# facebookresearch/sound-spaces

Hardware: AMD Instinct MI355X
Metric: audio env-steps/sec (RIR-convolve+spectrogram) per node, 128 envs Replica 16 kHz (higher is better)
Workload: dtype f32

## Files before the change

### include/ss_hip.h

```cpp
#ifndef SS_HIP_H
#define SS_HIP_H

#include <stddef.h>

#ifdef __cplusplus
extern "C" {
#endif

#define SS_EINVAL (-1)
#define SS_PAD_REFLECT 0
#define SS_PAD_CONSTANT 1
#define SS_FLAG_NO_DISTRACTOR 1
#define SS_FLAG_CROSSFADE 2
#define SS_FLAG_FIRST_BUCKET 4

int ss_block_len(void);
int ss_spec_floats(void);
int ss_version(void);

int ss_init(void);
int ss_release_scratch(void);

int ss_source_windows_f32(const float* src, const int* win_desc, float* spec_out, int n_windows,
                          void* stream);
// ... 202 lines not shown
    int* free_slots;
    int n_free;
    float* bank;
    long long bank_unit_stride;
    int bank_chan_stride, cap;
    int* dev_len;
    int* host_len;
    unsigned char* clipped;
    unsigned char* spec_stale;
    int keep;
    float* stage;
    int* stage_slot;
    int* stage_len;
    int* stage_desc;
    int stage_rows, threads;
    const unsigned char* used;
    const long long* use_seq;
    int* evicted_slot;
    int n_evicted, evict_cap;
    long long* loaded_key;
    int* loaded_slot;
    int* loaded_frames;
    int n_loaded, loaded_cap;
} ss_miss_loader;
int ss_ctx_observe_requests_load(ss_ctx* ctx, const long long* recs, int n, ss_request_tables* tables, ss_miss_loader* loader,
                                 float* audiogoal, float* spectrogram, int* miss_out, int* n_miss, void* stream);
int ss_ctx_load_rir_files(ss_ctx* ctx, ss_miss_loader* loader, const char* const* paths, int k, long long* last_used,
                          long long tick, int n_slots, void* stream);
int ss_ctx_requests_units(ss_ctx* ctx, const long long* recs, int n, const ss_request_tables* tables, int* units_out,
                          int* miss_out, int* n_miss);
int ss_ctx_plan(ss_ctx* ctx, const ss_units* units, int n, int* unit_desc_out, int* flags_out, int* n_new_windows_out,
                int* new_windows_out, int new_windows_cap);
int ss_ctx_stats(ss_ctx* ctx, long long* out8);

int ss_wav_read_rirs_f32(const char* const* paths, int n, float* dst, long long row_stride, int cap, int keep, int planar,
                         int* kept_out, int* frames_out, int* status_out, int n_threads);
int ss_bank_scatter_rows_f32(const float* staged, long long staged_row_stride, const int* slots, const int* lens, int n,
                             float* bank, long long unit_stride, int chan_stride, int cap, int* bank_len, void* stream);
int ss_bank_scatter_spectra_f32(const float* staged, long long staged_row_stride, int planar, const int* slots, const int* lens,
                                int n, float* hspec, int h_blocks, int* bank_len, void* stream);
int ss_bank_scatter_spectra16_f32(const float* staged, long long staged_row_stride, int planar, const int* slots, const int* lens,
                                  int n, void* hspec16, float* hscale, int h_blocks, int* bank_len, void* stream);
int ss_rows_gather_f32(const float* const* src, const int* n_floats, int n, float* dst, long long row_stride, int row_floats,
                       int n_threads);

#ifdef __cplusplus
}
#endif
#endif
```

### sound-spaces_amd/build.py

```python
#!/usr/bin/env python
import os
import subprocess
import sys

HERE = os.path.dirname(os.path.abspath(__file__))
CSRC = os.path.join(HERE, "csrc")
SO = os.path.join(CSRC, "libss_hip.so")
TORCH_SO = os.path.join(CSRC, "libss_torch_ops.so")
SOURCES = ["ss_torch_ops.cpp", "ss_hip.hip", "ss_kernels.hpp", "ss_fft_core.hpp", "ss_kernels32.hpp", "ss_fft_core32.hpp", "ss_features.hpp", "ss_tables.hpp", "ss_context.hpp", "ss_wavio.hpp", os.path.join("..", "..", "include", "ss_hip.h")]
FLAGS = ["--offload-arch=gfx950", "-O3", "-std=c++17", "-fPIC", "-shared", "-Wall", "-Wno-unused-function"]


STAMP = os.path.join(CSRC, ".libss_hip.srchash")
KERNEL_SOURCES = [s for s in SOURCES if s != "ss_torch_ops.cpp"]
KERNEL_STAMP = os.path.join(CSRC, ".libss_hip.kernelhash")


def _source_hash(sources=None):
    import hashlib
    h = hashlib.sha256(" ".join(FLAGS).encode())
    for s in (SOURCES if sources is None else sources):
        with open(os.path.join(CSRC, s), "rb") as f:
            h.update(f.read())
    return h.hexdigest()


def kernel_hash():
    return _source_hash(KERNEL_SOURCES)


def up_to_date():
    if not (os.path.exists(SO) and os.path.exists(STAMP)):
        return False
    if not os.path.exists(TORCH_SO) and not os.path.exists(TORCH_SO + ".skipped"):
        return False
    return open(STAMP).read().strip() == _source_hash()


def build(force=False, verbose=True):
    build_bench_token(force, verbose)
    if not force and up_to_date():
        if not os.path.exists(KERNEL_STAMP):
# ... 83 lines not shown
```

### sound-spaces_amd/csrc/ss_context.hpp

```cpp
#pragma once
#include <hip/hip_runtime.h>

#include <cstdint>
#include <cstring>
#include <unordered_map>
#include <vector>

#include "../../include/ss_hip.h"

namespace ssctx {

constexpr int kDirectDescUnits = 256;
constexpr int kRing = 16;
constexpr int kGroup = 4;
constexpr int kGuardTicks = 8;
constexpr int kLanes = 4;

inline int ceil_div(int a, int b) { return (a + b - 1) / b; }
inline int hip_rc(hipError_t e) { return e == hipSuccess ? 0 : -static_cast<int>(e); }

struct WindowSet {
    int m_min = 0, count = 0;
};

inline WindowSet plan_window_set(int source_len, long long t0, int nbh_max, int nby, bool wrap, int kb) {
    const long long limit = wrap ? 2LL * source_len : source_len;
    WindowSet ws;
    bool any = false;
    for (int m = -(nbh_max - 1); m <= nby - 1; ++m) {
        if (t0 + (long long)(m + 1) * kb > 0 && t0 + (long long)(m - 1) * kb < limit) {
            if (!any) { ws.m_min = m; any = true; }
            ++ws.count;
        }
    }
    return ws;
}

struct Entry {
    uint64_t key = 0;
    int m_min = 0, count = 0;
    long long tick = -1;
// ... 3 lines not shown

struct Context {
    int sr = 0, n_valid = 0, out_len = 0, pad_mode = 0, wrap_mode = 0, kb = 0, spec_floats = 0;
    int device = 0;
    float* src_dev = nullptr;
    size_t src_cap = 0, src_used = 0;
    std::vector<int> src_off, src_len;
    const float* rir = nullptr;
    const int* rir_len = nullptr;
    long long rir_us = 0;
    int rir_cs = 0, rir_es = 1, rir_cap = 0;
    const float* hspec = nullptr;
    const float* hscale = nullptr;
    int h_blocks = 0;
    std::vector<ss_rir_bucket> buckets;
    std::vector<ss_spec_bucket> spec_buckets;
    int stride = 1;
    int n_entries = 0;
    int pool_entries = 0;
    float* pool = nullptr;
    std::vector<Entry> entries;
    std::unordered_map<uint64_t, int> map;
    int lru_head = -1, lru_tail = -1;
    std::vector<int> free_list;
    long long tick = 0;
    long long hits = 0, misses = 0, evictions = 0, grows = 0;
    int ring_cap = 0, ring_k = 0;
    int* h_desc = nullptr;
    int* d_desc = nullptr;
    int win_cap = 0;
    int* h_win = nullptr;
    int* d_win = nullptr;
    hipEvent_t ev_done[kRing / kGroup] = {};
    bool group_open = false;
    int open_group = 0;
    hipStream_t group_stream = nullptr;
    bool ev_made = false;
    float* ag_scratch = nullptr;
    size_t ag_cap = 0;
    std::vector<int> sim_scratch;
    std::vector<int> new_win;
    std::vector<int> new_entries;
    bool plan_only_keys = false;
    hipStream_t last_stream = nullptr;
    bool have_last_stream = false;
    hipEvent_t ev_xstream = nullptr;
    int n_lanes = 1, lane_next = 0;
    void* miss_ev = nullptr;
    int spectral_max_units = 0;
    int mel_fused_min_units = 1, mel_fused_max_units = 0x7fffffff;
    int mel_rows_min_units = 1, mel_rows_max_units = 0;
    int mel_ss2_min_units = 1, mel_ss2_max_units = 0;
    int chip_share = 0;
    hipStream_t lane_stream[kLanes] = {};
    bool lane_dirty[kLanes] = {};
    bool lane_joined[kLanes] = {};
    bool lane_join_valid[kLanes] = {};
    hipStream_t lane_join_stream[kLanes] = {};
    hipEvent_t ev_lane[kLanes] = {};
    hipEvent_t ev_in = nullptr;
    hipEvent_t ev_win[kLanes] = {};
    long long win_seq[kLanes] = {};
    long long win_seen[kLanes][kLanes] = {};
    hipEvent_t ev_done_l[kLanes][kRing / kGroup] = {};
    bool lanes_made = false;
};

inline uint64_t make_key(int sound, long long t0, bool wrap) {
    return (static_cast<uint64_t>(static_cast<uint32_t>(sound)) << 33) |
// ... 172 lines not shown
```

### sound-spaces_amd/csrc/ss_hip.hip

```cpp
#include <hip/hip_runtime.h>

#include <algorithm>
#include <chrono>
#include <cstdlib>
#include <iterator>
#include <map>
#include <mutex>
#include <utility>
#include <new>
#include <string>
#include <vector>

#include "../../include/ss_hip.h"
#include "ss_context.hpp"
#include "ss_kernels.hpp"
#include "ss_kernels32.hpp"
#include "ss_features.hpp"
#include "ss_tables.hpp"
#include "ss_wavio.hpp"

namespace {

constexpr int kMaxDevices = 64;
struct DeviceTables {
// ... 39 lines not shown
    hipError_t e = hipGetDevice(&dev);
    if (e != hipSuccess) return hip_err(e);
    if (dev < 0 || dev >= kMaxDevices) return SS_EINVAL;
    std::lock_guard<std::mutex> lk(g_mu);
    DeviceTables& d = g_tables[dev];
    if (!d.ready) {
        const std::vector<float> host = ssk_host::build_tables();
        float* dev_buf = nullptr;
        e = hipMalloc(&dev_buf, host.size() * sizeof(float));
        if (e != hipSuccess) return hip_err(e);
        e = hipMemcpy(dev_buf, host.data(), host.size() * sizeof(float), hipMemcpyHostToDevice);
        if (e != hipSuccess) { (void)hipFree(dev_buf); return hip_err(e); }
        d.tb.twM = reinterpret_cast<const ssk::c32*>(dev_buf + ssk_host::kTwMOff);
        d.tb.twItem = reinterpret_cast<const ssk::c32*>(dev_buf + ssk_host::kTwItemOff);
        d.tb.tw512 = reinterpret_cast<const ssk::c32*>(dev_buf + ssk_host::kTw512Off);
        d.tb.win = dev_buf + ssk_host::kWinOff;
        d.tb.twG = reinterpret_cast<const ssk::c32*>(dev_buf + ssk_host::kTwGOff);
        d.tb.twP2 = reinterpret_cast<const ssk::c32*>(dev_buf + ssk_host::kTwP2Off);
        int cus = 0;
        e = hipDeviceGetAttribute(&cus, hipDeviceAttributeMultiprocessorCount, dev);
        if (e != hipSuccess) { (void)hipFree(dev_buf); return hip_err(e); }
        d.n_cus = cus > 0 ? cus : 1;
        d.ready = true;
    }
    *out = d.tb;
    if (n_cus) *n_cus = d.n_cus;
    return 0;
}

inline int n_frames_of(int len) { return 1 + len / ssk::kHop; }
inline int t4_of(int len) { return (n_frames_of(len) + ssk::kPool - 1) / ssk::kPool; }

thread_local const int* g_host_desc = nullptr;
thread_local int g_launch_share = 1;

inline bool fill_unit_tab(ssk::UnitTab<true>& ut, const int* host_desc, int n_units) {
    if (!host_desc || n_units > ssk::kTabUnits) return false;
    static const bool no_sort = ab_flag("SS_HIP_NO_SORT");
    unsigned key[ssk::kTabUnits];
    bool sortable = !no_sort && n_units >= 64;
    for (int i = 0; i < n_units; ++i) {
        const int* d = host_desc + 8 * i;
        const bool ok = d[0] >= 0 && d[2] <= 0 && d[2] + d[3] > 0;
        const int slot = ok ? d[1] - d[2] : 0xffffff;
        if (slot < 0 || slot > 0xffffff) sortable = false;
        key[i] = (static_cast<unsigned>(slot & 0xffffff) << 8) | static_cast<unsigned>(i);
    }
    if (sortable) std::sort(key, key + n_units);
    for (int k = 0; k < n_units; ++k) {
        const int i = sortable ? static_cast<int>(key[k] & 0xffu) : k;
        const int* d = host_desc + 8 * i;
        const bool ok = d[0] >= 0 && d[2] <= 0 && d[2] + d[3] > 0;
        ut.tab[ssk::kTabWords * k] = ok ? d[0] : -1;
        ut.tab[ssk::kTabWords * k + 1] = ok ? d[1] - d[2] : 0;
        ut.tab[ssk::kTabWords * k + 2] = i;
    }
    return true;
}

inline bool wide_one_block_ok(int out_len, int n_valid, int flags, bool spectral = false) {
    static const bool off = ab_flag("SS_HIP_NO_WIDE");
    if (off || spectral || out_len <= ssk::kB || n_valid < 0 || n_valid > ssk::kB) return false;
    if ((flags & SS_FLAG_CROSSFADE) &&
        (static_cast<int>(0.05 * out_len) < 1 || static_cast<int>(0.05 * out_len) > 2 * ssk::kPrevPairs - 2)) return false;
    return ssk::live_blocks(n_valid, out_len, t4_of(out_len)) <= 26;
}

inline int parts_log2_for(int n_rows, int n_cus) {
    static const int forced = ab_int("SS_HIP_PARTS_LOG2", -1);
    if (forced >= 0) return forced < 3 ? forced : 3;
    const int cus = n_cus / (g_launch_share > 1 ? g_launch_share : 1);
    int k = 0;
    while (k < 3 && (n_rows << (k + 1)) <= cus) ++k;
    return k;
}

template <bool FUSE>
int launch_conv(ssk::ConvParams p, int n_units, int nb_y, int flags, int n_cus, hipStream_t st, bool wide = false) {
    if (nb_y < 1 || nb_y > 3 || (FUSE && nb_y != 1)) return SS_EINVAL;
    p.nb_y = nb_y;
    p.parts_log2 = FUSE && !wide ? parts_log2_for(2 * n_units, n_cus) : 0;
    if constexpr (FUSE) {
        if (wide) {
            if ((flags & SS_FLAG_CROSSFADE) && (p.fade_len < 1 || p.fade_len > 2 * ssk::kPrevPairs - 2)) return SS_EINVAL;
            const dim3 grid(2 * n_units, 1), block(ssk::kT);
            if (flags & SS_FLAG_CROSSFADE)
                hipLaunchKernelGGL((ssk::k_conv<true, false, true, false, true>), grid, block, 0, st, p, ssk::UnitTab<false>());
            else
                hipLaunchKernelGGL((ssk::k_conv<true, false, false, false, true>), grid, block, 0, st, p, ssk::UnitTab<false>());
// ... 1044 lines not shown
    return launch_obs_rows<true, true, true>(p, n_units, flags, n_cus, static_cast<hipStream_t>(stream), m, ssk::SpecScale<true>{hscale});
}

struct ss_ctx { ssctx::Context c; };

int ss_ctx_create(ss_ctx** out, int sampling_rate, int n_valid, int pad_mode, int wrap_mode, int max_window_sets) {
    if (!out || sampling_rate <= 0 || n_valid < 0 || n_valid > sampling_rate || n_valid > 3 * ssk::kB) return SS_EINVAL;
    if (pad_mode != SS_PAD_REFLECT && pad_mode != SS_PAD_CONSTANT) return SS_EINVAL;
    ss_ctx* h = new (std::nothrow) ss_ctx();
    if (!h) return SS_EINVAL;
    ssctx::Context& c = h->c;
    c.sr = sampling_rate; c.n_valid = n_valid; c.out_len = sampling_rate; c.pad_mode = pad_mode;
    c.wrap_mode = wrap_mode ? 1 : 0;
    c.kb = ssk::kB; c.spec_floats = 2 * ssk::kSpecComplex;
    c.n_entries = max_window_sets > 0 ? max_window_sets : 256;
    c.stride = n_valid > 0 ? ssctx::ceil_div(n_valid, ssk::kB) : 1;
    ssctx::cache_reset(c);
    *out = h;
    return 0;
}

static void ctx_free_device(ssctx::Context& c) {
    if (c.pool) (void)hipFree(c.pool);
    if (c.src_dev) (void)hipFree(c.src_dev);
    if (c.d_desc) (void)hipFree(c.d_desc);
    if (c.d_win) (void)hipFree(c.d_win);
    if (c.h_desc) (void)hipHostFree(c.h_desc);
    if (c.h_win) (void)hipHostFree(c.h_win);
    if (c.ag_scratch) (void)hipFree(c.ag_scratch);
    c.ag_scratch = nullptr; c.ag_cap = 0;
    drop_wave_scratch(&c);
    if (c.ev_made)
        for (int k = 0; k < ssctx::kRing / ssctx::kGroup; ++k) (void)hipEventDestroy(c.ev_done[k]);
    if (c.ev_xstream) (void)hipEventDestroy(c.ev_xstream);
    if (c.miss_ev) { (void)hipEventDestroy(static_cast<hipEvent_t>(c.miss_ev)); c.miss_ev = nullptr; }
    c.ev_xstream = nullptr; c.have_last_stream = false;
    if (c.lanes_made) {
        for (int l = 0; l < ssctx::kLanes; ++l) {
            (void)hipStreamSynchronize(c.lane_stream[l]);
            drop_stash(c.lane_stream[l]);
            (void)hipEventDestroy(c.ev_lane[l]);
            (void)hipEventDestroy(c.ev_win[l]);
            (void)hipStreamDestroy(c.lane_stream[l]);
        }
        (void)hipEventDestroy(c.ev_in);
        for (int l = 1; l < ssctx::kLanes; ++l)
            for (int k = 0; k < ssctx::kRing / ssctx::kGroup; ++k) (void)hipEventDestroy(c.ev_done_l[l][k]);
        c.lanes_made = false;
    }
    c.pool = nullptr; c.src_dev = nullptr; c.d_desc = nullptr; c.d_win = nullptr; c.h_desc = nullptr; c.h_win = nullptr;
    c.ev_made = false;
}

int ss_ctx_destroy(ss_ctx* h) {
    if (!h) return 0;
    ctx_free_device(h->c);
    delete h;
    return 0;
}

int ss_ctx_add_source(ss_ctx* h, const float* clip, int len, int on_device) {
    if (!h || !clip || len <= 0) return SS_EINVAL;
    ssctx::Context& c = h->c;
    const size_t need = c.src_used + static_cast<size_t>(len);
    if (need > c.src_cap) {
        size_t cap = c.src_cap ? c.src_cap : (1u << 20);
// ... 86 lines not shown
int ss_ctx_set_rir_spectra16_rows(ss_ctx* h, const void* hspec16, const float* hscale, int h_blocks) {
    if (!h) return SS_EINVAL;
    ssctx::Context& c = h->c;
    if (!hspec16) {
        if (c.hscale) { c.hspec = nullptr; c.hscale = nullptr; c.h_blocks = 0; }
        return 0;
    }
    if (!hscale || h_blocks < 1 || h_blocks > 16 || (reinterpret_cast<size_t>(hspec16) & 7)) return SS_EINVAL;
    if (c.out_len <= c.kb || c.out_len > 3 * c.kb) return SS_EINVAL;
    if (c.rir || !c.buckets.empty() || !c.spec_buckets.empty() || !c.rir_len || (c.hspec && !c.hscale)) return SS_EINVAL;
    if (h_blocks != (c.rir_cap > 0 ? ssctx::ceil_div(c.rir_cap, c.kb) : 1)) return SS_EINVAL;
    c.hspec = static_cast<const float*>(hspec16);
    c.hscale = hscale;
    c.h_blocks = h_blocks;
    return 0;
}

int ss_ctx_plan(ss_ctx* h, const ss_units* units, int n, int* unit_desc_out, int* flags_out, int* n_new_windows_out,
                int* new_windows_out, int new_windows_cap) {
    if (!h || !unit_desc_out) return SS_EINVAL;
    ssctx::PlanResult res;
    int rc = ssctx::plan_units(h->c, units, n, unit_desc_out, &res);
    if (rc) return rc;
    h->c.plan_only_keys = true;
    if (flags_out) *flags_out = res.flags;
    if (n_new_windows_out) *n_new_windows_out = res.n_new_windows;
    if (new_windows_out) {
        const int k = res.n_new_windows < new_windows_cap ? res.n_new_windows : new_windows_cap;
        std::memcpy(new_windows_out, h->c.new_win.data(), sizeof(int) * 5 * static_cast<size_t>(k));
    }
    return 0;
}

int ss_ctx_stats(ss_ctx* h, long long* out8) {
    if (!h || !out8) return SS_EINVAL;
    const ssctx::Context& c = h->c;
    out8[0] = c.hits; out8[1] = c.misses; out8[2] = c.evictions; out8[3] = c.grows;
    out8[4] = c.n_entries; out8[5] = static_cast<long long>(c.map.size()); out8[6] = c.stride; out8[7] = c.tick;
    return 0;
}

static int ctx_ensure_ring(ssctx::Context& c, int n, int n_win, hipStream_t st) {
    hipError_t e;
    if (!c.ev_made) {
        for (int k = 0; k < ssctx::kRing / ssctx::kGroup; ++k) {
            e = hipEventCreateWithFlags(&c.ev_done[k], hipEventDisableTiming);
            if (e != hipSuccess) return hip_err(e);
        }
        c.ev_made = true;
    }
    if (n > c.ring_cap) {
        e = hipDeviceSynchronize();
        if (e != hipSuccess) return hip_err(e);
        int cap = c.ring_cap ? c.ring_cap : 256;
        while (cap < n) cap *= 2;
        if (c.h_desc) (void)hipHostFree(c.h_desc);
        if (c.d_desc) (void)hipFree(c.d_desc);
        c.h_desc = nullptr; c.d_desc = nullptr; c.ring_cap = 0;
        const size_t bytes = sizeof(int) * 8 * static_cast<size_t>(cap) * ssctx::kRing;
        e = hipHostMalloc(reinterpret_cast<void**>(&c.h_desc), bytes, hipHostMallocDefault);
        if (e != hipSuccess) return hip_err(e);
        e = hipMalloc(reinterpret_cast<void**>(&c.d_desc), bytes);
        if (e != hipSuccess) return hip_err(e);
        c.ring_cap = cap;
    }
    if (n_win > c.win_cap) {
        e = hipDeviceSynchronize();
        if (e != hipSuccess) return hip_err(e);
        int cap = c.win_cap ? c.win_cap : 256;
        while (cap < n_win) cap *= 2;
        if (c.h_win) (void)hipHostFree(c.h_win);
        if (c.d_win) (void)hipFree(c.d_win);
        c.h_win = nullptr; c.d_win = nullptr; c.win_cap = 0;
        const size_t bytes = sizeof(int) * 5 * static_cast<size_t>(cap) * ssctx::kRing;
        e = hipHostMalloc(reinterpret_cast<void**>(&c.h_win), bytes, hipHostMallocDefault);
        if (e != hipSuccess) return hip_err(e);
        e = hipMalloc(reinterpret_cast<void**>(&c.d_win), bytes);
        if (e != hipSuccess) return hip_err(e);
        c.win_cap = cap;
    }
    (void)st;
// ... 18 lines not shown
}

static int ctx_observe_on(ss_ctx* h, const ss_units* units, int n, float* audiogoal, float* spectrogram, void* stream,
                          int lane, const ss_features* mel = nullptr) {
    ssctx::Context& c = h->c;
    hipStream_t st = static_cast<hipStream_t>(stream);
    hipError_t e;
    SS_PROF_BEGIN();
    if (c.plan_only_keys) {
        e = hipDeviceSynchronize();
        if (e != hipSuccess) return hip_err(e);
        ssctx::cache_reset(c);
        c.plan_only_keys = false;
    }
    if (lane >= 0) {
        for (int o = 0; o < c.n_lanes; ++o) {
            if (o == lane || c.win_seen[lane][o] >= c.win_seq[o]) continue;
            e = hipStreamWaitEvent(st, c.ev_win[o], 0);
            if (e != hipSuccess) return hip_err(e);
            c.win_seen[lane][o] = c.win_seq[o];
        }
    } else if (c.have_last_stream && st != c.last_stream) {
        if (!c.ev_xstream) {
            e = hipEventCreateWithFlags(&c.ev_xstream, hipEventDisableTiming);
            if (e != hipSuccess) return hip_err(e);
        }
        e = hipEventRecord(c.ev_xstream, c.last_stream);
        if (e == hipSuccess) e = hipStreamWaitEvent(st, c.ev_xstream, 0);
        if (e != hipSuccess) return hip_err(e);
    }
    SS_PROF_MARK(1);
    int rc = ctx_ensure_ring(c, n, 0, st);
    if (rc) return rc;
    if (lane < 0 && c.group_open && (st != c.group_stream || c.ring_k / ssctx::kGroup != c.open_group)) {
        e = hipEventRecord(c.ev_done[c.open_group], c.group_stream);
        if (e != hipSuccess) return hip_err(e);
        c.group_open = false;
        c.ring_k = (c.open_group + 1) * ssctx::kGroup % ssctx::kRing;
    }
    const int k = c.ring_k, g = k / ssctx::kGroup;
    if (k % ssctx::kGroup == 0) {
        e = hipEventSynchronize(c.ev_done[g]);
        for (int l = 1; lane >= 0 && l < c.n_lanes && e == hipSuccess; ++l) e = hipEventSynchronize(c.ev_done_l[l][g]);
        if (e != hipSuccess) return hip_err(e);
        c.group_open = lane < 0;
        c.group_stream = st;
        c.open_group = g;
    }
    static const bool force_copy = ab_flag("SS_HIP_DESC_COPY");
    const bool direct = !force_copy && n <= ssctx::kDirectDescUnits;
    int* hd = c.h_desc + static_cast<size_t>(k) * c.ring_cap * 8;
    int* dd = direct ? hd : c.d_desc + static_cast<size_t>(k) * c.ring_cap * 8;
    ssctx::PlanResult res;
    SS_PROF_MARK(2);
    rc = ssctx::plan_units(c, units, n, hd, &res);
    if (rc) return rc;
    const bool spec_bk = !c.spec_buckets.empty();
    if (!c.rir && c.buckets.empty() && ((!c.hspec && !spec_bk) || (res.flags & SS_FLAG_CROSSFADE))) {
        ssctx::cache_rollback(c);
        return SS_EINVAL;
    }
    SS_PROF_MARK(3);
    c.ring_k = (k + 1) % ssctx::kRing;
    auto close_slot = [&]() -> int {
        hipError_t ee = hipSuccess;
        if (lane >= 0) {
            if (k % ssctx::kGroup >= ssctx::kGroup - c.n_lanes) ee = hipEventRecord(lane == 0 ? c.ev_done[g] : c.ev_done_l[lane][g], st);
        } else if (k % ssctx::kGroup == ssctx::kGroup - 1) {
            ee = hipEventRecord(c.ev_done[g], st);
            c.group_open = false;
        }
        return hip_err(ee);
    };
    auto fail = [&](int code) { ssctx::cache_rollback(c); (void)close_slot(); return code; };
    rc = ctx_ensure_pool(c, st);
    if (rc) return fail(rc);
    if (res.n_new_windows > 0) {
        rc = ctx_ensure_ring(c, n, res.n_new_windows, st);
        if (rc) return fail(rc);
        int* hw = c.h_win + static_cast<size_t>(k) * c.win_cap * 5;
        int* dw = c.d_win + static_cast<size_t>(k) * c.win_cap * 5;
        std::memcpy(hw, c.new_win.data(), sizeof(int) * 5 * static_cast<size_t>(res.n_new_windows));
        e = hipMemcpyAsync(dw, hw, sizeof(int) * 5 * static_cast<size_t>(res.n_new_windows), hipMemcpyHostToDevice, st);
        if (e != hipSuccess) return fail(hip_err(e));
        rc = launch_windows_scatter(c.src_dev, dw, c.pool, res.n_new_windows, st);
        if (rc) return fail(rc);
        if (lane >= 0) {
            e = hipEventRecord(c.ev_win[lane], st);
            if (e != hipSuccess) return fail(hip_err(e));
            ++c.win_seq[lane];
        }
    }
    c.new_entries.clear();
    c.last_stream = st;
    c.have_last_stream = true;
    if (!direct) {
        e = hipMemcpyAsync(dd, hd, sizeof(int) * 8 * static_cast<size_t>(n), hipMemcpyHostToDevice, st);
        if (e != hipSuccess) return fail(hip_err(e));
    }
    const bool spectral = (c.hspec || spec_bk) && !(res.flags & SS_FLAG_CROSSFADE) &&
                          !(c.spectral_max_units > 0 && c.rir && c.out_len <= ssk::kB && n > c.spectral_max_units &&
                            (res.flags & SS_FLAG_NO_DISTRACTOR));
    const int nbh_bank = spectral && !spec_bk ? c.h_blocks : (c.rir_cap > 0 ? ssctx::ceil_div(c.rir_cap, c.kb) : 1);
    const bool mel_fused = mel && c.buckets.empty() && !spec_bk && obs_logmel_shape_ok(c.out_len, res.flags) &&
                           n >= c.mel_fused_min_units && n <= c.mel_fused_max_units;
    const bool mel_rows = mel && !mel_fused && (!c.hscale || c.out_len > c.kb) && c.buckets.empty() && !spec_bk && (spectral || (c.rir && c.rir_cap > 0)) &&
                          obs_logmel_rows_shape_ok(c.out_len, c.n_valid, nbh_bank, res.flags) &&
                          n >= c.mel_rows_min_units && n <= c.mel_rows_max_units;
    const bool mel_ss2 = mel && !mel_fused && !mel_rows && c.buckets.empty() && c.rir && !spectral &&
                         obs_logmel_ss2_shape(c.out_len, c.n_valid, res.flags) != 0 &&
                         n >= c.mel_ss2_min_units && n <= c.mel_ss2_max_units;
    if (mel && !mel_fused && !mel_rows && !mel_ss2) {
        rc = get_wave_scratch(&c, lane < 0 ? 0 : lane, st, static_cast<size_t>(n) * 2 * c.out_len, &audiogoal);
        if (rc) return fail(rc);
    }
    if (spectrogram && !audiogoal && !mel_rows && c.out_len > ssk::kB && !wide_one_block_ok(c.out_len, c.n_valid, res.flags, spectral) &&
        !obs_rows_ok(c.out_len, c.n_valid, nbh_bank, res.flags, spectral, true)) {
        const size_t need = static_cast<size_t>(n) * 2 * c.out_len;
        if (need > c.ag_cap) {
            e = hipDeviceSynchronize();
            if (e != hipSuccess) return fail(hip_err(e));
            if (c.ag_scratch) (void)hipFree(c.ag_scratch);
            c.ag_scratch = nullptr; c.ag_cap = 0;
            e = hipMalloc(reinterpret_cast<void**>(&c.ag_scratch), need * sizeof(float));
            if (e != hipSuccess) return fail(hip_err(e));
            c.ag_cap = need;
        }
        audiogoal = c.ag_scratch;
    }
    static const bool no_tab = ab_flag("SS_HIP_NO_UNIT_TAB");
    SS_PROF_MARK(4);
    g_host_desc = no_tab ? nullptr : hd;
    g_launch_share = c.chip_share > 0 ? c.chip_share : c.n_lanes;
    if (mel_ss2) {
        rc = ss_audio_obs_logmel_ss2_f32(c.pool, c.rir, c.rir_len, dd, nullptr, spectrogram, mel->logmel, mel->mel_start, mel->mel_w,
                                         mel->n_mels, mel->max_len, mel->mel_eps, n, c.rir_us, c.rir_cs, c.rir_es, c.rir_cap,
                                         c.n_valid, c.out_len, c.pad_mode, res.flags, stream);
    } else if (mel_rows) {
        rc = spectral && c.hscale
                 ? ss_audio_obs_logmel_rows_spec16_f32(c.pool, c.hspec, c.hscale, c.rir_len, dd, nullptr, spectrogram, mel->logmel,
                                                       mel->mel_start, mel->mel_w, mel->n_mels, mel->max_len, mel->mel_eps, n,
                                                       c.h_blocks, c.n_valid, c.out_len, c.pad_mode, res.flags, stream)
             : spectral ? ss_audio_obs_logmel_rows_spec_f32(c.pool, c.hspec, c.rir_len, dd, nullptr, spectrogram, mel->logmel,
                                                          mel->mel_start, mel->mel_w, mel->n_mels, mel->max_len, mel->mel_eps, n,
                                                          c.h_blocks, c.n_valid, c.out_len, c.pad_mode, res.flags, stream)
                      : ss_audio_obs_logmel_rows_f32(c.pool, c.rir, c.rir_len, dd, nullptr, spectrogram, mel->logmel, mel->mel_start,
                                                     mel->mel_w, mel->n_mels, mel->max_len, mel->mel_eps, n, c.rir_us, c.rir_cs,
                                                     c.rir_es, c.rir_cap, c.n_valid, c.out_len, c.pad_mode, res.flags, stream);
    } else if (mel_fused) {
        rc = spectral && c.hscale
                 ? ss_audio_obs_logmel_spec16_f32(c.pool, c.hspec, c.hscale, c.rir_len, dd, nullptr, spectrogram, mel->logmel,
                                                  mel->mel_start, mel->mel_w, mel->n_mels, mel->max_len, mel->mel_eps, n, c.h_blocks,
                                                  c.n_valid, c.out_len, c.pad_mode, res.flags, stream)
             : spectral ? ss_audio_obs_logmel_spec_f32(c.pool, c.hspec, c.rir_len, dd, nullptr, spectrogram, mel->logmel, mel->mel_start,
                                                     mel->mel_w, mel->n_mels, mel->max_len, mel->mel_eps, n, c.h_blocks, c.n_valid,
                                                     c.out_len, c.pad_mode, res.flags, stream)
                      : ss_audio_obs_logmel_f32(c.pool, c.rir, c.rir_len, dd, nullptr, spectrogram, mel->logmel, mel->mel_start,
                                                mel->mel_w, mel->n_mels, mel->max_len, mel->mel_eps, n, c.rir_us, c.rir_cs, c.rir_es,
                                                c.rir_cap, c.n_valid, c.out_len, c.pad_mode, res.flags, stream);
    } else if (spec_bk) {
        const int nb = static_cast<int>(c.spec_buckets.size());
        rc = spectrogram ? ss_audio_obs_spec_buckets_f32(c.pool, c.spec_buckets.data(), nb, c.rir_len, dd, audiogoal, spectrogram, n,
                                                         c.n_valid, c.out_len, c.pad_mode, res.flags, stream)
                         : ss_fftconv_binaural_spec_buckets_f32(c.pool, c.spec_buckets.data(), nb, c.rir_len, dd, audiogoal, n,
                                                                c.n_valid, c.out_len, res.flags, stream);
    } else if (!c.buckets.empty()) {
        const int nb = static_cast<int>(c.buckets.size());
        rc = spectrogram ? ss_audio_obs_buckets_f32(c.pool, c.buckets.data(), nb, c.rir_len, dd, audiogoal, spectrogram, n,
                                                    c.n_valid, c.out_len, c.pad_mode, res.flags, stream)
                         : ss_fftconv_binaural_buckets_f32(c.pool, c.buckets.data(), nb, c.rir_len, dd, audiogoal, n, c.n_valid,
                                                           c.out_len, res.flags, stream);
    } else if (spectrogram && spectral && c.hscale && c.out_len > c.kb)
        rc = ss_audio_obs_rows_spec16_f32(c.pool, c.hspec, c.hscale, c.rir_len, dd, audiogoal, spectrogram, n, c.h_blocks, c.n_valid,
                                          c.out_len, c.pad_mode, res.flags, stream);
    else if (spectrogram && spectral && c.hscale)
        rc = ss_audio_obs_spec16_f32(c.pool, c.hspec, c.hscale, c.rir_len, dd, audiogoal, spectrogram, n, c.h_blocks, c.n_valid,
                                     c.out_len, c.pad_mode, res.flags, stream);
    else if (spectral && c.hscale)
        rc = ss_fftconv_binaural_spec16_f32(c.pool, c.hspec, c.hscale, c.rir_len, dd, audiogoal, n, c.h_blocks, c.n_valid, c.out_len,
                                            res.flags, stream);
    else if (spectrogram && spectral)
        rc = ss_audio_obs_spec_f32(c.pool, c.hspec, c.rir_len, dd, audiogoal, spectrogram, n, c.h_blocks, c.n_valid,
                                   c.out_len, c.pad_mode, res.flags, stream);
    else if (spectrogram)
        rc = ss_audio_obs_f32(c.pool, c.rir, c.rir_len, dd, audiogoal, spectrogram, n, c.rir_us, c.rir_cs, c.rir_es,
                              c.rir_cap, c.n_valid, c.out_len, c.pad_mode, res.flags, stream);
    else if (spectral)
        rc = ss_fftconv_binaural_spec_f32(c.pool, c.hspec, c.rir_len, dd, audiogoal, n, c.h_blocks, c.n_valid, c.out_len,
                                          res.flags, stream);
    else
        rc = ss_fftconv_binaural_f32(c.pool, c.rir, c.rir_len, dd, audiogoal, n, c.rir_us, c.rir_cs, c.rir_es, c.rir_cap,
                                     c.n_valid, c.out_len, res.flags, stream);
    g_host_desc = nullptr;
    g_launch_share = 1;
    SS_PROF_MARK(5);
    if (!rc && mel && !mel_fused && !mel_rows && !mel_ss2)
        rc = ss_audio_features_f32(audiogoal, n, c.out_len, c.pad_mode, nullptr, mel->logmel, mel->mel_start, mel->mel_w,
                                   mel->n_mels, mel->max_len, mel->mel_eps, nullptr, 1, 1.f, stream);
    if (rc) return fail(rc);
    rc = close_slot();
    SS_PROF_MARK(6);
    return rc;
}

int ss_ctx_set_overlap(ss_ctx* h, int n_streams) {
    if (!h || n_streams < 1 || n_streams > ssctx::kLanes) return SS_EINVAL;
    ssctx::Context& c = h->c;
    hipError_t e = hipDeviceSynchronize();
    if (e != hipSuccess) return hip_err(e);
    if (n_streams > 1 && !c.lanes_made) {
        for (int l = 0; l < ssctx::kLanes; ++l) {
            e = hipStreamCreateWithFlags(&c.lane_stream[l], hipStreamNonBlocking);
            if (e == hipSuccess) e = hipEventCreateWithFlags(&c.ev_lane[l], hipEventDisableTiming);
            if (e == hipSuccess) e = hipEventCreateWithFlags(&c.ev_win[l], hipEventDisableTiming);
            if (e != hipSuccess) return hip_err(e);
        }
        e = hipEventCreateWithFlags(&c.ev_in, hipEventDisableTiming);
        if (e != hipSuccess) return hip_err(e);
        for (int k = 0; k < ssctx::kRing / ssctx::kGroup; ++k) {
            for (int l = 1; l < ssctx::kLanes; ++l) {
                e = hipEventCreateWithFlags(&c.ev_done_l[l][k], hipEventDisableTiming);
                if (e != hipSuccess) return hip_err(e);
            }
        }
        c.lanes_made = true;
    }
    c.n_lanes = n_streams;
    c.lane_next = 0;
    c.ring_k = 0;
    c.group_open = false;
    c.have_last_stream = false;
    for (int l = 0; l < ssctx::kLanes; ++l) { c.lane_dirty[l] = false; c.lane_joined[l] = false; c.lane_join_valid[l] = false; for (int o = 0; o < ssctx::kLanes; ++o) c.win_seen[l][o] = c.win_seq[o]; }
    return 0;
}

int ss_ctx_set_spectral_policy(ss_ctx* h, int max_units) {
    if (!h || max_units < 0) return SS_EINVAL;
    h->c.spectral_max_units = max_units;
    return 0;
}

int ss_ctx_set_logmel_policy(ss_ctx* h, int min_units, int max_units) {
    if (!h || min_units < 0 || max_units < 0) return SS_EINVAL;
    h->c.mel_fused_min_units = min_units;
    h->c.mel_fused_max_units = max_units;
    return 0;
}

int ss_ctx_set_logmel_rows_policy(ss_ctx* h, int min_units, int max_units) {
    if (!h || min_units < 0 || max_units < 0) return SS_EINVAL;
    h->c.mel_rows_min_units = min_units;
    h->c.mel_rows_max_units = max_units;
    return 0;
}

int ss_ctx_set_logmel_ss2_policy(ss_ctx* h, int min_units, int max_units) {
    if (!h || min_units < 0 || max_units < 0) return SS_EINVAL;
    h->c.mel_ss2_min_units = min_units;
    h->c.mel_ss2_max_units = max_units;
    return 0;
}

size_t ss_ctx_wave_scratch_bytes(const ss_ctx* h) {
// ... 871 lines not shown
```

### sound-spaces_amd/ss_amd/_lib.py

```python
from __future__ import annotations

import ctypes
import os

_HERE = os.path.dirname(os.path.abspath(__file__))
SO_PATH = os.path.normpath(os.path.join(_HERE, "..", "csrc", "libss_hip.so"))

EXPORTS = ("ss_block_len", "ss_spec_floats", "ss_version", "ss_init", "ss_source_windows_f32",
           "ss_fftconv_binaural_f32", "ss_spectrogram_f32", "ss_audio_obs_f32", "ss_intensity_f32", "ss_logmel_f32", "ss_gccphat_f32",
           "ss_ctx_create", "ss_ctx_destroy", "ss_ctx_add_source", "ss_ctx_add_source_len", "ss_ctx_set_rir_bank",
           "ss_ctx_observe", "ss_ctx_plan", "ss_ctx_stats", "ss_ctx_set_rir_spectra",
           "ss_rir_spectra_f32", "ss_fftconv_binaural_spec_f32", "ss_audio_obs_spec_f32", "ss_ctx_observe_sims",
           "ss_ctx_sims_units", "ss_ctx_set_overlap", "ss_ctx_join", "ss_fftconv_binaural_buckets_f32",
           "ss_audio_obs_buckets_f32", "ss_ctx_set_rir_buckets", "ss_release_scratch",
           "ss_source_windows32_f32", "ss_audio_obs32_f32", "ss_ctx_observe_requests", "ss_ctx_requests_units", "ss_audio_features_f32", "ss_ctx_observe_features",
           "ss_wav_read_rirs_f32", "ss_rows_gather_f32", "ss_bank_scatter_rows_f32", "ss_ctx_set_chip_share", "ss_ctx_set_spectral_policy", "ss_ctx_observe_requests_load", "ss_ctx_load_rir_files",
           "ss_bank_scatter_spectra_f32", "ss_audio_obs_logmel_f32", "ss_audio_obs_logmel_spec_f32", "ss_ctx_set_logmel_policy",
           "ss_audio_obs_logmel_rows_f32", "ss_audio_obs_logmel_rows_spec_f32", "ss_ctx_set_logmel_rows_policy",
           "ss_audio_obs_logmel_ss2_f32", "ss_ctx_set_logmel_ss2_policy",
           "ss_rir_spectra16_f32", "ss_bank_scatter_spectra16_f32", "ss_fftconv_binaural_spec16_f32", "ss_audio_obs_spec16_f32",
           "ss_audio_obs_logmel_spec16_f32", "ss_ctx_set_rir_spectra16",
           "ss_audio_obs_rows_spec16_f32", "ss_audio_obs_logmel_rows_spec16_f32", "ss_ctx_set_rir_spectra16_rows",
           "ss_fftconv_binaural_spec_buckets_f32", "ss_audio_obs_spec_buckets_f32", "ss_ctx_set_rir_spec_buckets")
EXPORTS_SIZE = ("ss_ctx_wave_scratch_bytes",)


class SsRirBucket(ctypes.Structure):
    _fields_ = [("rir", ctypes.c_void_p), ("hspec", ctypes.c_void_p), ("first", ctypes.c_int), ("n_entries", ctypes.c_int),
                ("cap", ctypes.c_int), ("reserved", ctypes.c_int)]


class SsSpecBucket(ctypes.Structure):
    _fields_ = [("hspec", ctypes.c_void_p), ("hscale", ctypes.c_void_p), ("first", ctypes.c_int), ("n_entries", ctypes.c_int),
                ("cap", ctypes.c_int), ("reserved", ctypes.c_int)]


class SsMissLoader(ctypes.Structure):
    _fields_ = [("table_dirs", ctypes.POINTER(ctypes.c_char_p)), ("n_table_dirs", ctypes.c_int),
                ("pair_keys", ctypes.c_void_p), ("pair_slots", ctypes.c_void_p), ("pair_cap", ctypes.c_int),
                ("free_slots", ctypes.c_void_p), ("n_free", ctypes.c_int),
                ("bank", ctypes.c_void_p), ("bank_unit_stride", ctypes.c_longlong), ("bank_chan_stride", ctypes.c_int),
                ("cap", ctypes.c_int), ("dev_len", ctypes.c_void_p), ("host_len", ctypes.c_void_p), ("clipped", ctypes.c_void_p),
                ("spec_stale", ctypes.c_void_p), ("keep", ctypes.c_int),
                ("stage", ctypes.c_void_p), ("stage_slot", ctypes.c_void_p), ("stage_len", ctypes.c_void_p),
# ... 34 lines not shown
class SsHipError(RuntimeError):
    pass


def load() -> ctypes.CDLL:
    global _lib
    if _lib is not None:
        return _lib
    if not os.path.exists(SO_PATH):
        raise SsHipError(f"{SO_PATH} not found: build it with `python sound-spaces_amd/build.py` "
                         "(or __graft_entry__.build()); there is no CPU fallback for this path")
    lib = ctypes.CDLL(SO_PATH)
    c_int, c_ll, vp = ctypes.c_int, ctypes.c_longlong, ctypes.c_void_p
    lib.ss_block_len.restype = c_int
    lib.ss_spec_floats.restype = c_int
    lib.ss_version.restype = c_int
    lib.ss_init.restype = c_int
    lib.ss_source_windows_f32.argtypes = [vp, vp, vp, c_int, vp]
    lib.ss_fftconv_binaural_f32.argtypes = [vp, vp, vp, vp, vp, c_int, c_ll, c_int, c_int, c_int, c_int, c_int, c_int, vp]
    lib.ss_spectrogram_f32.argtypes = [vp, vp, c_int, c_int, c_int, vp]
    lib.ss_audio_obs_f32.argtypes = [vp, vp, vp, vp, vp, vp, c_int, c_ll, c_int, c_int, c_int, c_int, c_int, c_int, c_int, vp]
    lib.ss_intensity_f32.argtypes = [vp, vp, c_int, c_int, c_int, vp]
    lib.ss_gccphat_f32.argtypes = [vp, vp, c_int, c_int, c_int, c_int, ctypes.c_float, vp]
    lib.ss_logmel_f32.argtypes = [vp, vp, c_int, c_int, c_int, vp, vp, c_int, c_int, ctypes.c_float, vp]
    pp = ctypes.POINTER(ctypes.c_void_p)
    lib.ss_ctx_create.argtypes = [pp, c_int, c_int, c_int, c_int, c_int]
    lib.ss_ctx_destroy.argtypes = [vp]
    lib.ss_ctx_add_source.argtypes = [vp, vp, c_int, c_int]
    lib.ss_ctx_add_source_len.argtypes = [vp, c_int]
    lib.ss_ctx_set_rir_bank.argtypes = [vp, vp, vp, c_ll, c_int, c_int, c_int]
    lib.ss_ctx_observe.argtypes = [vp, ctypes.POINTER(SsUnits), c_int, vp, vp, vp]
    lib.ss_ctx_plan.argtypes = [vp, ctypes.POINTER(SsUnits), c_int, vp, vp, vp, vp, c_int]
    lib.ss_ctx_stats.argtypes = [vp, vp]
    lib.ss_ctx_observe_sims.argtypes = [vp, ctypes.POINTER(SsSimColumns), c_int, vp, vp, vp, vp, vp]
    lib.ss_ctx_sims_units.argtypes = [vp, ctypes.POINTER(SsSimColumns), c_int, vp, vp, vp]
    lib.ss_ctx_set_rir_spectra.argtypes = [vp, vp, c_int]
    lib.ss_ctx_set_overlap.argtypes = [vp, c_int]
    lib.ss_fftconv_binaural_buckets_f32.argtypes = [vp, vp, c_int, vp, vp, vp, c_int, c_int, c_int, c_int, vp]
    lib.ss_audio_obs_buckets_f32.argtypes = [vp, vp, c_int, vp, vp, vp, vp, c_int, c_int, c_int, c_int, c_int, vp]
    lib.ss_ctx_set_rir_buckets.argtypes = [vp, vp, c_int, vp]
    lib.ss_ctx_join.argtypes = [vp, vp]
    lib.ss_ctx_set_chip_share.argtypes = [vp, c_int]
    lib.ss_ctx_set_spectral_policy.argtypes = [vp, c_int]
    lib.ss_rir_spectra_f32.argtypes = [vp, vp, c_int, c_ll, c_int, c_int, vp]
    lib.ss_fftconv_binaural_spec_f32.argtypes = [vp, vp, vp, vp, vp, c_int, c_int, c_int, c_int, c_int, vp]
    lib.ss_audio_obs_spec_f32.argtypes = [vp, vp, vp, vp, vp, vp, c_int, c_int, c_int, c_int, c_int, c_int, vp]
    lib.ss_audio_obs_logmel_f32.argtypes = [vp, vp, vp, vp, vp, vp, vp, vp, vp, c_int, c_int, ctypes.c_float, c_int, c_ll, c_int, c_int,
                                            c_int, c_int, c_int, c_int, c_int, vp]
    lib.ss_audio_obs_logmel_spec_f32.argtypes = [vp, vp, vp, vp, vp, vp, vp, vp, vp, c_int, c_int, ctypes.c_float, c_int, c_int, c_int,
                                                 c_int, c_int, c_int, vp]
    lib.ss_ctx_set_logmel_policy.argtypes = [vp, c_int, c_int]
    lib.ss_audio_obs_logmel_rows_f32.argtypes = lib.ss_audio_obs_logmel_f32.argtypes
    lib.ss_audio_obs_logmel_rows_spec_f32.argtypes = lib.ss_audio_obs_logmel_spec_f32.argtypes
    lib.ss_ctx_set_logmel_rows_policy.argtypes = [vp, c_int, c_int]
    lib.ss_audio_obs_logmel_ss2_f32.argtypes = lib.ss_audio_obs_logmel_f32.argtypes
    lib.ss_ctx_set_logmel_ss2_policy.argtypes = [vp, c_int, c_int]
    lib.ss_ctx_wave_scratch_bytes.argtypes = [vp]
    lib.ss_source_windows32_f32.argtypes = [vp, vp, vp, c_int, vp]
    lib.ss_audio_obs32_f32.argtypes = [vp, vp, vp, vp, vp, vp, c_int, c_ll, c_int, c_int, c_int, c_int, c_int, c_int, vp]
    lib.ss_audio_features_f32.argtypes = [vp, c_int, c_int, c_int, vp, vp, vp, vp, c_int, c_int, ctypes.c_float, vp, c_int,
                                          ctypes.c_float, vp]
    lib.ss_ctx_observe_features.argtypes = [vp, ctypes.POINTER(SsUnits), c_int, vp, vp, ctypes.POINTER(SsFeatures), vp]
    lib.ss_ctx_observe_requests.argtypes = [vp, vp, c_int, vp, vp, vp, vp, vp, vp]
    lib.ss_ctx_requests_units.argtypes = [vp, vp, c_int, vp, vp, vp, vp]
    lib.ss_ctx_observe_requests_load.argtypes = [vp, vp, c_int, vp, vp, vp, vp, vp, vp, vp]
    lib.ss_ctx_load_rir_files.argtypes = [vp, vp, vp, c_int, vp, c_ll, c_int, vp]
# ... 58 lines not shown
```

### sound-spaces_amd/ss_amd/context.py

```python
from __future__ import annotations

import ctypes
from typing import Dict, Optional

import numpy as np

from . import _lib
from .planning import spectrogram_shape

_PAD = {"reflect": 0, "constant": 1, 0: 0, 1: 1}


def _col(a, dtype):
    if a is None:
        return None
    a = np.ascontiguousarray(a, dtype=dtype)
    return a


_NO_MISS = np.zeros((0,), np.int32)


class AudioContext:
    def __init__(self, sampling_rate: int, step_time: Optional[float] = None, wrap: bool = False,
# ... 312 lines not shown
        if rc != 0:
            _lib.check(rc, "ss_ctx_observe_requests")
        return miss["n"].value

    def observe_requests_load(self, recs: bytes, n: int, tables, loader, spectrogram_ptr, audiogoal_ptr, stream: int, miss) -> int:
        rc = self.lib.ss_ctx_observe_requests_load(self._h, recs, n, tables["ref"], loader["ref"], audiogoal_ptr, spectrogram_ptr,
                                                   miss["ptr"], miss["n_ptr"], stream)
        if rc != 0:
            _lib.check(rc, "ss_ctx_observe_requests_load")
        return miss["n"].value

    def requests_units(self, recs: bytes, n: int, tables):
        out = np.zeros((5, max(n, 1)), np.int32)
        miss, n_miss = np.zeros((max(n, 1),), np.int32), ctypes.c_int(0)
        _lib.check(self.lib.ss_ctx_requests_units(self._h, recs, n, tables["ref"], out.ctypes.data, miss.ctypes.data,
                                                  ctypes.addressof(n_miss)), "ss_ctx_requests_units")
        return dict(zip(("sound", "t0", "rir", "dis_sound", "dis_rir"), out[:, :n])), miss[:min(n_miss.value, n)].copy()

    def plan(self, sound, t0, rir, dis_sound=None, dis_rir=None, last_rir=None, wrap=None, last_wrap=None):
        u, n, keep = self._units(sound, t0, rir, dis_sound, dis_rir, last_rir, wrap, last_wrap)
        desc = np.zeros((n, 8), np.int32)
        flags, nw = ctypes.c_int(0), ctypes.c_int(0)
        cap = 2 * self.stats()["slots_per_key"] * n + 16
        wins = np.zeros((cap, 5), np.int32)
        _lib.check(self.lib.ss_ctx_plan(self._h, ctypes.byref(u), n, desc.ctypes.data, ctypes.addressof(flags),
                                        ctypes.addressof(nw), wins.ctypes.data, cap), "ss_ctx_plan")
        assert nw.value <= cap
        return desc, flags.value, wins[:nw.value]

    def stats(self) -> Dict[str, int]:
        out = np.zeros(8, np.int64)
        _lib.check(self.lib.ss_ctx_stats(self._h, out.ctypes.data), "ss_ctx_stats")
        keys = ("hits", "misses", "evictions", "grows", "capacity", "resident", "slots_per_key", "steps")
        return dict(zip(keys, (int(v) for v in out)))
```

Measured before the change: 4.695 million.

## Skip ring-slot release events when slots unread and add pacing event

Moves descriptor-ring group release logic into a Release helper that records a group's done event only if some slot in the group was actually read by the device, and only waits on groups that were recorded. When the unit table was passed by value and no new windows were staged, the slot counts as unread, so the event record and later host synchronize are skipped. A separate Pace event is recorded every kRing steps, with a host wait on the previous one, to bound how far the host runs ahead once ring events stop being recorded. Counters are exposed through a new ring-stats API, and the risk is a subtle reuse hazard if the slot_read tracking misses a case where the device still reads the slot.

```diff
diff --git a/include/ss_hip.h b/include/ss_hip.h
--- a/include/ss_hip.h
+++ b/include/ss_hip.h
@@ -258,6 +258,7 @@
 int ss_ctx_plan(ss_ctx* ctx, const ss_units* units, int n, int* unit_desc_out, int* flags_out, int* n_new_windows_out,
                 int* new_windows_out, int new_windows_cap);
 int ss_ctx_stats(ss_ctx* ctx, long long* out8);
+int ss_ctx_ring_stats(ss_ctx* ctx, long long* out4);
 
 int ss_wav_read_rirs_f32(const char* const* paths, int n, float* dst, long long row_stride, int cap, int keep, int planar,
                          int* kept_out, int* frames_out, int* status_out, int n_threads);
diff --git a/sound-spaces_amd/build.py b/sound-spaces_amd/build.py
--- a/sound-spaces_amd/build.py
+++ b/sound-spaces_amd/build.py
@@ -7,7 +7,7 @@
 CSRC = os.path.join(HERE, "csrc")
 SO = os.path.join(CSRC, "libss_hip.so")
 TORCH_SO = os.path.join(CSRC, "libss_torch_ops.so")
-SOURCES = ["ss_torch_ops.cpp", "ss_hip.hip", "ss_kernels.hpp", "ss_fft_core.hpp", "ss_kernels32.hpp", "ss_fft_core32.hpp", "ss_features.hpp", "ss_tables.hpp", "ss_context.hpp", "ss_wavio.hpp", os.path.join("..", "..", "include", "ss_hip.h")]
+SOURCES = ["ss_torch_ops.cpp", "ss_hip.hip", "ss_kernels.hpp", "ss_fft_core.hpp", "ss_kernels32.hpp", "ss_fft_core32.hpp", "ss_features.hpp", "ss_tables.hpp", "ss_context.hpp", "ss_ring.hpp", "ss_wavio.hpp", os.path.join("..", "..", "include", "ss_hip.h")]
 FLAGS = ["--offload-arch=gfx950", "-O3", "-std=c++17", "-fPIC", "-shared", "-Wall", "-Wno-unused-function"]
 
 
diff --git a/sound-spaces_amd/csrc/ss_context.hpp b/sound-spaces_amd/csrc/ss_context.hpp
--- a/sound-spaces_amd/csrc/ss_context.hpp
+++ b/sound-spaces_amd/csrc/ss_context.hpp
@@ -7,6 +7,7 @@
 #include <vector>
 
 #include "../../include/ss_hip.h"
+#include "ss_ring.hpp"
 
 namespace ssctx {
 
@@ -76,9 +77,10 @@
     int* h_win = nullptr;
     int* d_win = nullptr;
     hipEvent_t ev_done[kRing / kGroup] = {};
-    bool group_open = false;
-    int open_group = 0;
+    ssring::Release<kRing, kGroup> ring;
     hipStream_t group_stream = nullptr;
+    ssring::Pace<kRing> pace;
+    hipEvent_t ev_pace = nullptr;
     bool ev_made = false;
     float* ag_scratch = nullptr;
     size_t ag_cap = 0;
diff --git a/sound-spaces_amd/csrc/ss_hip.hip b/sound-spaces_amd/csrc/ss_hip.hip
--- a/sound-spaces_amd/csrc/ss_hip.hip
+++ b/sound-spaces_amd/csrc/ss_hip.hip
@@ -95,6 +95,7 @@
 inline int t4_of(int len) { return (n_frames_of(len) + ssk::kPool - 1) / ssk::kPool; }
 
 thread_local const int* g_host_desc = nullptr;
+thread_local bool g_tab_taken = false;
 thread_local int g_launch_share = 1;
 
 inline bool fill_unit_tab(ssk::UnitTab<true>& ut, const int* host_desc, int n_units) {
@@ -118,6 +119,7 @@
         ut.tab[ssk::kTabWords * k + 1] = ok ? d[1] - d[2] : 0;
         ut.tab[ssk::kTabWords * k + 2] = i;
     }
+    g_tab_taken = true;
     return true;
 }
 
@@ -1228,6 +1230,7 @@
     drop_wave_scratch(&c);
     if (c.ev_made)
         for (int k = 0; k < ssctx::kRing / ssctx::kGroup; ++k) (void)hipEventDestroy(c.ev_done[k]);
+    if (c.ev_pace) { (void)hipEventDestroy(c.ev_pace); c.ev_pace = nullptr; }
     if (c.ev_xstream) (void)hipEventDestroy(c.ev_xstream);
     if (c.miss_ev) { (void)hipEventDestroy(static_cast<hipEvent_t>(c.miss_ev)); c.miss_ev = nullptr; }
     c.ev_xstream = nullptr; c.have_last_stream = false;
@@ -1380,6 +1383,13 @@
     return 0;
 }
 
+int ss_ctx_ring_stats(ss_ctx* h, long long* out4) {
+    if (!h || !out4) return SS_EINVAL;
+    out4[0] = h->c.ring.n_records; out4[1] = h->c.ring.n_waits;
+    out4[2] = h->c.pace.n_records; out4[3] = h->c.pace.n_waits;
+    return 0;
+}
+
 int ss_ctx_stats(ss_ctx* h, long long* out8) {
     if (!h || !out8) return SS_EINVAL;
     const ssctx::Context& c = h->c;
@@ -1395,6 +1405,8 @@
             e = hipEventCreateWithFlags(&c.ev_done[k], hipEventDisableTiming);
             if (e != hipSuccess) return hip_err(e);
         }
+        e = hipEventCreateWithFlags(&c.ev_pace, hipEventDisableTiming);
+        if (e != hipSuccess) return hip_err(e);
         c.ev_made = true;
     }
     if (n > c.ring_cap) {
@@ -1479,20 +1491,26 @@
     SS_PROF_MARK(1);
     int rc = ctx_ensure_ring(c, n, 0, st);
     if (rc) return rc;
-    if (lane < 0 && c.group_open && (st != c.group_stream || c.ring_k / ssctx::kGroup != c.open_group)) {
-        e = hipEventRecord(c.ev_done[c.open_group], c.group_stream);
+    if (lane < 0 && c.ring.must_close_before(c.ring_k, st == c.group_stream)) {
+        const int og = c.ring.open_group;
+        if (c.ring.close_early()) {
+            e = hipEventRecord(c.ev_done[og], c.group_stream);
+            if (e != hipSuccess) return hip_err(e);
+        }
+        c.ring_k = c.ring.next_slot();
+    }
+    const int k = c.ring_k, g = k / ssctx::kGroup;
+    if (lane < 0) {
+        if (c.ring.begin(k)) {
+            e = hipEventSynchronize(c.ev_done[g]);
+            if (e != hipSuccess) return hip_err(e);
+        }
+        if (k % ssctx::kGroup == 0) c.group_stream = st;
+    } else if (k % ssctx::kGroup == 0) {
+        e = hipEventSynchronize(c.ev_done[g]);
+        for (int l = 1; l < c.n_lanes && e == hipSuccess; ++l) e = hipEventSynchronize(c.ev_done_l[l][g]);
         if (e != hipSuccess) return hip_err(e);
-        c.group_open = false;
-        c.ring_k = (c.open_group + 1) * ssctx::kGroup % ssctx::kRing;
-    }
-    const int k = c.ring_k, g = k / ssctx::kGroup;
-    if (k % ssctx::kGroup == 0) {
-        e = hipEventSynchronize(c.ev_done[g]);
-        for (int l = 1; lane >= 0 && l < c.n_lanes && e == hipSuccess; ++l) e = hipEventSynchronize(c.ev_done_l[l][g]);
-        if (e != hipSuccess) return hip_err(e);
-        c.group_open = lane < 0;
-        c.group_stream = st;
-        c.open_group = g;
+        ++c.ring.n_waits;
     }
     static const bool force_copy = ab_flag("SS_HIP_DESC_COPY");
     const bool direct = !force_copy && n <= ssctx::kDirectDescUnits;
@@ -1509,13 +1527,23 @@
     }
     SS_PROF_MARK(3);
     c.ring_k = (k + 1) % ssctx::kRing;
+    bool slot_read = true;
     auto close_slot = [&]() -> int {
         hipError_t ee = hipSuccess;
         if (lane >= 0) {
-            if (k % ssctx::kGroup >= ssctx::kGroup - c.n_lanes) ee = hipEventRecord(lane == 0 ? c.ev_done[g] : c.ev_done_l[lane][g], st);
-        } else if (k % ssctx::kGroup == ssctx::kGroup - 1) {
+            if (k % ssctx::kGroup >= ssctx::kGroup - c.n_lanes) {
+                ee = hipEventRecord(lane == 0 ? c.ev_done[g] : c.ev_done_l[lane][g], st);
+                ++c.ring.n_records;
+            }
+        } else if (c.ring.end(k, slot_read)) {
             ee = hipEventRecord(c.ev_done[g], st);
-            c.group_open = false;
+            c.pace.ring_event();
+        } else {
+            bool wait_first = false;
+            if (c.pace.step(&wait_first)) {
+                if (wait_first) ee = hipEventSynchronize(c.ev_pace);
+                if (ee == hipSuccess) ee = hipEventRecord(c.ev_pace, st);
+            }
         }
         return hip_err(ee);
     };
@@ -1578,6 +1606,7 @@
     static const bool no_tab = ab_flag("SS_HIP_NO_UNIT_TAB");
     SS_PROF_MARK(4);
     g_host_desc = no_tab ? nullptr : hd;
+    g_tab_taken = false;
     g_launch_share = c.chip_share > 0 ? c.chip_share : c.n_lanes;
     if (mel_ss2) {
         rc = ss_audio_obs_logmel_ss2_f32(c.pool, c.rir, c.rir_len, dd, nullptr, spectrogram, mel->logmel, mel->mel_start, mel->mel_w,
@@ -1640,6 +1669,7 @@
                                      c.n_valid, c.out_len, res.flags, stream);
     g_host_desc = nullptr;
     g_launch_share = 1;
+    slot_read = !direct || res.n_new_windows > 0 || !g_tab_taken;
     SS_PROF_MARK(5);
     if (!rc && mel && !mel_fused && !mel_rows && !mel_ss2)
         rc = ss_audio_features_f32(audiogoal, n, c.out_len, c.pad_mode, nullptr, mel->logmel, mel->mel_start, mel->mel_w,
@@ -1675,7 +1705,8 @@
     c.n_lanes = n_streams;
     c.lane_next = 0;
     c.ring_k = 0;
-    c.group_open = false;
+    c.ring.reset();
+    c.pace.reset();
     c.have_last_stream = false;
     for (int l = 0; l < ssctx::kLanes; ++l) { c.lane_dirty[l] = false; c.lane_joined[l] = false; c.lane_join_valid[l] = false; for (int o = 0; o < ssctx::kLanes; ++o) c.win_seen[l][o] = c.win_seq[o]; }
     return 0;
diff --git a/sound-spaces_amd/csrc/ss_ring.hpp b/sound-spaces_amd/csrc/ss_ring.hpp
--- /dev/null
+++ b/sound-spaces_amd/csrc/ss_ring.hpp
@@ -0,0 +1,62 @@
+#pragma once
+
+namespace ssring {
+
+template <int RING, int GROUP>
+struct Release {
+    static constexpr int kGroups = RING / GROUP;
+    bool recorded[kGroups] = {};
+    bool open = false;
+    bool open_read = false;
+    int open_group = 0;
+    long long n_records = 0, n_waits = 0;
+
+    void reset() {
+        for (int g = 0; g < kGroups; ++g) recorded[g] = false;
+        open = open_read = false;
+    }
+    bool must_close_before(int k, bool same_stream) const { return open && (!same_stream || k / GROUP != open_group); }
+    bool close_early() {
+        const bool rec = open_read;
+        if (rec) { recorded[open_group] = true; ++n_records; }
+        open = open_read = false;
+        return rec;
+    }
+    int next_slot() const { return (open_group + 1) * GROUP % RING; }
+    bool begin(int k) {
+        if (k % GROUP) return false;
+        const int g = k / GROUP;
+        const bool wait = recorded[g];
+        if (wait) { recorded[g] = false; ++n_waits; }
+        open = true;
+        open_read = false;
+        open_group = g;
+        return wait;
+    }
+    bool end(int k, bool slot_read) {
+        open_read = open_read || slot_read;
+        if (k % GROUP != GROUP - 1) return false;
+        return close_early();
+    }
+};
+
+template <int PACE>
+struct Pace {
+    int since = 0;
+    bool recorded = false;
+    long long n_records = 0, n_waits = 0;
+
+    void reset() { since = 0; recorded = false; }
+    void ring_event() { since = 0; }
+    bool step(bool* wait_first) {
+        *wait_first = false;
+        if (++since < PACE) return false;
+        since = 0;
+        if (recorded) { *wait_first = true; ++n_waits; }
+        recorded = true;
+        ++n_records;
+        return true;
+    }
+};
+
+}
diff --git a/sound-spaces_amd/ss_amd/_lib.py b/sound-spaces_amd/ss_amd/_lib.py
--- a/sound-spaces_amd/ss_amd/_lib.py
+++ b/sound-spaces_amd/ss_amd/_lib.py
@@ -9,7 +9,7 @@
 EXPORTS = ("ss_block_len", "ss_spec_floats", "ss_version", "ss_init", "ss_source_windows_f32",
            "ss_fftconv_binaural_f32", "ss_spectrogram_f32", "ss_audio_obs_f32", "ss_intensity_f32", "ss_logmel_f32", "ss_gccphat_f32",
            "ss_ctx_create", "ss_ctx_destroy", "ss_ctx_add_source", "ss_ctx_add_source_len", "ss_ctx_set_rir_bank",
-           "ss_ctx_observe", "ss_ctx_plan", "ss_ctx_stats", "ss_ctx_set_rir_spectra",
+           "ss_ctx_observe", "ss_ctx_plan", "ss_ctx_stats", "ss_ctx_ring_stats", "ss_ctx_set_rir_spectra",
            "ss_rir_spectra_f32", "ss_fftconv_binaural_spec_f32", "ss_audio_obs_spec_f32", "ss_ctx_observe_sims",
            "ss_ctx_sims_units", "ss_ctx_set_overlap", "ss_ctx_join", "ss_fftconv_binaural_buckets_f32",
            "ss_audio_obs_buckets_f32", "ss_ctx_set_rir_buckets", "ss_release_scratch",
@@ -110,6 +110,7 @@
     lib.ss_ctx_observe.argtypes = [vp, ctypes.POINTER(SsUnits), c_int, vp, vp, vp]
     lib.ss_ctx_plan.argtypes = [vp, ctypes.POINTER(SsUnits), c_int, vp, vp, vp, vp, c_int]
     lib.ss_ctx_stats.argtypes = [vp, vp]
+    lib.ss_ctx_ring_stats.argtypes = [vp, vp]
     lib.ss_ctx_observe_sims.argtypes = [vp, ctypes.POINTER(SsSimColumns), c_int, vp, vp, vp, vp, vp]
     lib.ss_ctx_sims_units.argtypes = [vp, ctypes.POINTER(SsSimColumns), c_int, vp, vp, vp]
     lib.ss_ctx_set_rir_spectra.argtypes = [vp, vp, c_int]
diff --git a/sound-spaces_amd/ss_amd/context.py b/sound-spaces_amd/ss_amd/context.py
--- a/sound-spaces_amd/ss_amd/context.py
+++ b/sound-spaces_amd/ss_amd/context.py
@@ -368,4 +368,6 @@
         out = np.zeros(8, np.int64)
         _lib.check(self.lib.ss_ctx_stats(self._h, out.ctypes.data), "ss_ctx_stats")
         keys = ("hits", "misses", "evictions", "grows", "capacity", "resident", "slots_per_key", "steps")
-        return dict(zip(keys, (int(v) for v in out)))
+        ring = np.zeros(4, np.int64)
+        _lib.check(self.lib.ss_ctx_ring_stats(self._h, ring.ctypes.data), "ss_ctx_ring_stats")
+        return dict(zip(keys + ("ring_events", "ring_waits", "pace_events", "pace_waits"), (int(v) for v in (*out, *ring))))
```

Measured after the change: 4.760 million (median of 6 runs). +1.4%, better.
